# violetdenim/c3dgs

Hardware: AMD Instinct MI355X
Metric: raster views/sec fwd+bwd @1920x1080 (higher is better)
Workload: dtype f32; 1 GPU; BASELINE.json configs[2]: synth-v1 3M Gaussians, SH deg 3, indexed-camera rasterizer (QAT inner loop), mark_visible+fwd+bwd, 1 view/step/GPU; gaussians=3000000, width=1920, height=1080, sh_codebook=304096, gaussian_codebook=754096, parallelism=replicas x1

## Files before the change

c3dgs_amd/_lib.py:

```python
import ctypes as C
import os

_HERE = os.path.dirname(os.path.abspath(__file__))
LIB_PATH = os.environ.get("C3DGS_LIB_PATH") or os.path.join(_HERE, "libc3dgs_hip.so")

_f32p = C.POINTER(C.c_float)
_i64p = C.POINTER(C.c_int64)
_i32p = C.POINTER(C.c_int32)
_u8p = C.POINTER(C.c_uint8)

RESIZE_FN = C.CFUNCTYPE(C.c_void_p, C.c_void_p, C.c_size_t)


class RasterParams(C.Structure):
    _fields_ = [
        ("P", C.c_int32), ("D", C.c_int32), ("M", C.c_int32), ("W", C.c_int32), ("H", C.c_int32),
        ("SHS", C.c_int32), ("GS", C.c_int32),
        ("background", C.c_void_p), ("means3D", C.c_void_p), ("sh", C.c_void_p), ("colors_precomp", C.c_void_p),
        ("opacities", C.c_void_p), ("scales", C.c_void_p), ("scale_factors", C.c_void_p), ("rotations", C.c_void_p),
        ("cov3D_precomp", C.c_void_p), ("sh_indices", C.c_void_p), ("g_indices", C.c_void_p),
        ("viewmatrix", C.c_void_p), ("projmatrix", C.c_void_p), ("campos", C.c_void_p),
        ("tan_fovx", C.c_float), ("tan_fovy", C.c_float), ("scale_modifier", C.c_float),
        ("prefiltered", C.c_int32), ("clamp_color", C.c_int32), ("debug", C.c_int32),
    ]
# ... 10 lines not shown
        "total_bytes", "splat", "depth_keys", "depth_keys_sorted", "depth_order",
        "sorted_offsets", "inst_offset", "rects", "clamped", "scan_temp", "scan_temp_bytes", "block_base", "depth_base")]


class BinningLayout(C.Structure):
    _fields_ = [(n, C.c_size_t) for n in (
        "total_bytes", "keys_unsorted", "values_unsorted", "keys_sorted", "point_list", "sort_temp", "sort_temp_bytes")]


class StageTime(C.Structure):
    _fields_ = [("name", C.c_char * 32), ("total_ms", C.c_double), ("count", C.c_int64)]


class ImageLayout(C.Structure):
    _fields_ = [(n, C.c_size_t) for n in ("total_bytes", "final_T", "n_contrib", "ranges", "tile_used", "tile_order")]


class QatParams(C.Structure):
    _fields_ = [("P", C.c_int32), ("GS", C.c_int32), ("SHS", C.c_int32), ("M", C.c_int32),
                ("xyz", C.c_void_p), ("opacity", C.c_void_p), ("scaling_factor", C.c_void_p), ("scaling", C.c_void_p),
                ("rotation", C.c_void_p), ("features_dc", C.c_void_p), ("features_rest", C.c_void_p), ("state", C.c_void_p),
                ("observer_enabled", C.c_int32 * 6), ("fake_quant_enabled", C.c_int32 * 6),
                ("half_xyz", C.c_int32), ("averaging_constant", C.c_float)]


class AdamTensor(C.Structure):
    _fields_ = [("param", C.c_void_p), ("grad", C.c_void_p), ("exp_avg", C.c_void_p), ("exp_avg_sq", C.c_void_p), ("n", C.c_int64),
                ("step_size", C.c_float), ("bias_correction2_sqrt", C.c_float)]


# ... 56 lines not shown
    "c3dgs_qat_points": (C.c_int, [C.POINTER(QatParams)] + [_vp] * 10),
    "c3dgs_qat_points_backward": (C.c_int, [C.POINTER(QatParams)] + [_vp] * 11),
    "c3dgs_qat_quantize": (C.c_int, [C.POINTER(QatParams), C.c_int32] + [_vp] * 7),
    "c3dgs_fake_quantize": (C.c_int, [C.c_int64, _vp, _vp, C.c_int32, C.c_int32, C.c_float, _vp, _vp, _vp]),
    "c3dgs_fake_quantize_backward": (C.c_int, [C.c_int64, _vp, _vp, C.c_int32, _vp, _vp, _vp]),
    "c3dgs_debug_lane_counters": (C.c_int, [C.POINTER(C.c_uint64), _vp]),
    "c3dgs_debug_sort_times": (C.c_int, [C.POINTER(C.c_uint64)]),
    "c3dgs_debug_gather_probe": (C.c_int, [C.c_int32, C.c_int64, _vp, _vp, _vp, _vp]),
    "c3dgs_debug_sort_temp_bytes": (C.c_size_t, [C.c_int32, C.c_int64, C.c_int32]),
    "c3dgs_debug_sort_pairs": (C.c_int, [C.c_int32, C.c_int64, C.c_int32, _vp, _vp, _vp, _vp, _vp, C.c_size_t, _vp]),
    "c3dgs_debug_tile_sort_temp_bytes": (C.c_size_t, [C.c_int32, C.c_int64]),
    "c3dgs_debug_tile_sort_pairs": (C.c_int, [C.c_int32, C.c_int64, _vp, _vp, _vp, _vp, _vp, C.c_size_t, _vp]),
    "c3dgs_get_geom_layout": (C.c_int, [C.c_int32, C.POINTER(GeomLayout)]),
    "c3dgs_get_binning_layout": (C.c_int, [C.c_int32, C.c_int32, C.c_int32, C.POINTER(BinningLayout)]),
    "c3dgs_get_image_layout": (C.c_int, [C.c_int32, C.c_int32, C.POINTER(ImageLayout)]),
    "c3dgs_backward_workspace_bytes": (C.c_size_t, [C.c_int32, C.c_int32]),
    "c3dgs_profile_enable": (C.c_int, [C.c_int]),
    "c3dgs_profile_only": (C.c_int, [C.c_char_p]),
    "c3dgs_profile_read": (C.c_int, [C.POINTER(StageTime), C.c_int]),
    "c3dgs_last_error": (C.c_char_p, []),
    "c3dgs_abi_version": (C.c_int, []),
    "c3dgs_abs_accumulate": (C.c_int, [C.c_int64, C.c_void_p, C.c_void_p, C.c_void_p]),
}

_lib = None


def lib():
    global _lib
    if _lib is None:
# ... 32 lines not shown
```

c3dgs_amd/csrc/binning.hip:

```cpp
#include "common.hpp"
#include <rocprim/device/device_radix_sort.hpp>
#include <rocprim/iterator/counting_iterator.hpp>

namespace c3dgs {

size_t scan_temp_bytes(int P)
{
    size_t a = 0, b = 0;
    (void)rocprim::radix_sort_pairs(nullptr, b, (const uint32_t*)nullptr, (uint32_t*)nullptr, (const uint32_t*)nullptr,
                                    (uint32_t*)nullptr, (size_t)P, 0u, 32u);
    size_t m = a > b ? a : b;
    const size_t os = onesweep_depth_temp_bytes(P);
    if (os > m) m = os;
    return m < 256 ? 256 : m;
}

size_t sort_temp_bytes(int R, int end_bit, int key_bytes)
{
    size_t bytes = 0;
    if (key_bytes == 4)
        (void)rocprim::radix_sort_pairs(nullptr, bytes, (const uint32_t*)nullptr, (uint32_t*)nullptr,
                                        (const uint32_t*)nullptr, (uint32_t*)nullptr, (size_t)R, 0u, (unsigned)end_bit);
    else
        (void)rocprim::radix_sort_pairs(nullptr, bytes, (const uint16_t*)nullptr, (uint16_t*)nullptr,
                                        (const uint32_t*)nullptr, (uint32_t*)nullptr, (size_t)R, 0u, (unsigned)end_bit);
    const size_t os = onesweep_tile_temp_bytes(R, end_bit, key_bytes);
    if (os > bytes) bytes = os;
    const size_t reuse = align_up((size_t)(R > 0 ? R : 1));
    if (reuse > bytes) bytes = reuse;
    return bytes < 256 ? 256 : bytes;
}

__global__ void __launch_bounds__(256)
gather_u64_kernel(int n, const uint32_t* __restrict__ idx, const uint2* __restrict__ src, uint2* __restrict__ dst)
{
    const int i = blockIdx.x * 256 + threadIdx.x;
    if (i < n) dst[i] = src[idx[i]];
}

size_t depth_sort_clear_bytes(int P)
{
    return (onesweep_enabled() && (size_t)P < ((size_t)1 << 30)) ? onesweep_depth_clear_bytes(P) : 0;
}
// ... 34 lines not shown
```

c3dgs_amd/csrc/c_abi.hip:

```cpp
#include "common.hpp"
#include <cstdlib>
#include <cstring>
#include <mutex>
#include <vector>

namespace c3dgs {

static thread_local std::string g_last_error;
void set_error(const std::string& msg) { g_last_error = msg; }

enum Stage { ST_MARK_VISIBLE, ST_PREPROCESS, ST_DEPTH_SORT, ST_SCAN, ST_DUPLICATE, ST_SORT, ST_RANGES, ST_RENDER_FWD, ST_ZERO_PARTIALS,
             ST_RENDER_BWD, ST_BWD_PREPROCESS, ST_WDIST, ST_VQ_ACC, ST_VQ_APPLY, ST_LOSS_FWD, ST_LOSS_BWD,
             ST_QAT_OBSERVE, ST_QAT_CODEBOOKS, ST_QAT_VISIBLE, ST_QAT_POINTS, ST_QAT_POINTS_BWD, ST_QAT_CODEBOOKS_BWD, ST_ADAM,
             ST_KNN_SORT, ST_KNN_BOUNDS, ST_KNN_QUERY, ST_COUNT };
static const char* kStageNames[ST_COUNT] = { "mark_visible", "preprocess", "depth_sort", "scan", "duplicate_with_keys", "sort",
                                             "identify_ranges", "render_forward", "zero_partials", "render_backward",
                                             "backward_preprocess", "weighted_distance", "vq_accumulate", "vq_apply", "l1_ssim_forward",
                                             "l1_ssim_backward", "qat_observe", "qat_codebooks", "qat_visible", "qat_points",
                                             "qat_points_backward", "qat_codebooks_backward", "adam_step",
                                             "knn_sort", "knn_bounds", "knn_query" };
struct ProfRec { int stage; hipEvent_t a, b; };
static std::mutex g_prof_mu;
static bool g_prof_on = false;
static int g_prof_only = -1;
// ... 176 lines not shown
    if (R > 0) {
        const int end_bit = tile_sort_end_bit(W, H);
        size_t tclear = tile_sort_clear_bytes(R, end_bit, b.key_bytes);
        if (tclear > b.sort_temp_bytes) tclear = 0;
        { StageTimer t_(ST_DUPLICATE, s); launch_duplicate_with_keys(P, g, b, gx, sort_err, b.sort_temp, tclear / 16, s); }
        C3DGS_STAGE("duplicate_with_keys", p.debug, s);
        { StageTimer t_(ST_SORT, s);
          C3DGS_HIP_TRY(run_tile_sort(b.sort_temp, b.sort_temp_bytes, b.keys_unsorted, b.keys_sorted, b.key_bytes, b.values_unsorted,
                                      b.point_list, R, end_bit, s, tclear != 0)); }
        C3DGS_STAGE("sort", p.debug, s);
        if (p.debug && onesweep_timed_out(s)) return fail(C3DGS_E_HIP, "tile sort: look-back timed out");
        { StageTimer t_(ST_RANGES, s); launch_identify_ranges(R, b.keys_sorted, b.key_bytes, img.ranges, sort_err, s); }
        C3DGS_STAGE("identify_ranges", p.debug, s);
    }
    { StageTimer t_(ST_RENDER_FWD, s);
      launch_render_forward(W, H, img, b.point_list, g.splat, p.background, out_color, (uint8_t*)b.sort_temp, sort_err, s); }
    C3DGS_STAGE("render_forward", p.debug, s);
    return C3DGS_OK;
}

static int backward_impl(const c3dgs_raster_params* pp, bool indexed, const int32_t* radii, const void* geom_buffer,
                         const void* binning_buffer, const void* image_buffer, int32_t R, const float* dL_dout_color,
                         c3dgs_resize_fn ws_resize, void* ws_user, const c3dgs_raster_grads* grads, void* stream_)
{
    if (int rc = validate(pp, indexed, true)) return rc;
    if (!grads) return fail(C3DGS_E_INVALID, "grads is NULL");
    c3dgs_raster_params p = *pp;
    if (!indexed) { p.sh_indices = nullptr; p.g_indices = nullptr; p.scale_factors = nullptr; }
    hipStream_t s = (hipStream_t)stream_;
    const int P = p.P, W = p.W, H = p.H;

// ... 30 lines not shown
    float* partials = (float*)ws_resize(ws_user, ws_bytes);
    if (!partials) return fail(C3DGS_E_ALLOC, "backward workspace allocation failed");

    const size_t r1 = (size_t)(R > 0 ? R : 1), p256 = ((size_t)P + 1023) / 1024 * 1024;
    uint8_t* touched = (uint8_t*)partials + align_up(r1 * PARTIAL_FLOATS * sizeof(float));
    uint32_t* tile_order = img.tile_order;
    uint32_t* live_ids = (uint32_t*)(touched + align_up(r1)) + 65536;
    uint32_t* live_slots = live_ids + p256;
    uint32_t* live_count = live_slots + p256;
    { StageTimer t_(ST_ZERO_PARTIALS, s);
      launch_backward_prep(R > 0 ? W : 0, H, img, tile_order, touched, align_up(r1) / 16, R > 0 ? nullptr : cb_zero,
                           R > 0 ? 0 : cb_zero16, s); }
    if (R > 0) {
        const BinPtrs b = bin_ptrs(const_cast<void*>(binning_buffer), R, W, H);
        { StageTimer t_(ST_RENDER_BWD, s);
          launch_render_backward(W, H, img, b.point_list, g.splat, g.block_base, p.background, dL_dout_color, partials, touched,
                                 (const uint8_t*)b.sort_temp, tile_order, cb_zero, cb_zero16, s); }
        C3DGS_STAGE("render_backward", p.debug, s);
    }
    { StageTimer t_(ST_BWD_PREPROCESS, s);
      launch_backward_preprocess(p, radii, g, partials, touched, live_count, live_ids, live_slots, *grads, s); }
    C3DGS_STAGE("backward_preprocess", p.debug, s);
    return C3DGS_OK;
}

}

using namespace c3dgs;

extern "C" {

const char* c3dgs_last_error(void) { return g_last_error.c_str(); }
// ... 132 lines not shown
    geom_layout(P, out);
    return C3DGS_OK;
}
int c3dgs_get_binning_layout(int32_t R, int32_t W, int32_t H, c3dgs_binning_layout* out)
{
    if (!out || R < 0 || W <= 0 || H <= 0) return fail(C3DGS_E_INVALID, "bad arguments");
    binning_layout(R, W, H, out);
    return C3DGS_OK;
}
int c3dgs_get_image_layout(int32_t W, int32_t H, c3dgs_image_layout* out)
{
    if (!out || W <= 0 || H <= 0) return fail(C3DGS_E_INVALID, "bad arguments");
    image_layout(W, H, out);
    return C3DGS_OK;
}
size_t c3dgs_backward_workspace_bytes(int32_t P, int32_t R)
{
    const size_t r = (size_t)(R > 0 ? R : 1), p256 = ((size_t)(P > 0 ? P : 1) + 1023) / 1024 * 1024;
    return align_up(r * PARTIAL_FLOATS * sizeof(float)) + align_up(r) + 65536 * sizeof(uint32_t) +
           (2 * p256 + p256 / 256) * sizeof(uint32_t) + 256;
}

int c3dgs_mark_visible(int32_t P, const float* means3D, const float* viewmatrix, const float* projmatrix, uint8_t* present,
                       void* stream)
{
    (void)projmatrix;
    if (P < 0) return fail(C3DGS_E_INVALID, "P must be >= 0");
    if (P == 0) return C3DGS_OK;
    if (!means3D || !viewmatrix || !present) return fail(C3DGS_E_INVALID, "means3D, viewmatrix and present are required");
    { StageTimer t_(ST_MARK_VISIBLE, (hipStream_t)stream); launch_mark_visible(P, means3D, viewmatrix, present, (hipStream_t)stream); }
// ... 427 lines not shown
```

c3dgs_amd/csrc/common.hpp:

```cpp
#pragma once
#include <hip/hip_runtime.h>
#include <cstdint>
#include <cstddef>
#include <cstdio>
#include <cstring>
#include <string>

#include "../../include/c3dgs_hip.h"

namespace c3dgs {

constexpr int TILE = 16;
constexpr int TILE_PIX = 256;
constexpr int SPLAT_F4 = 3;
constexpr int PARTIAL_FLOATS = 9;

void set_error(const std::string& msg);
inline int fail(int code, const std::string& msg) { set_error(msg); return code; }

#define C3DGS_HIP_TRY(expr)                                                                         \
    do {                                                                                            \
        hipError_t e__ = (expr);                                                                    \
        if (e__ != hipSuccess)                                                                      \
            return ::c3dgs::fail(C3DGS_E_HIP, std::string(#expr) + ": " + hipGetErrorString(e__));  \
// ... 70 lines not shown

inline void binning_layout(int R, int W, int H, c3dgs_binning_layout* L)
{
    size_t o = 0, r = (size_t)(R > 0 ? R : 1);
    const int end_bit = tile_sort_end_bit(W, H);
    const size_t kb = (size_t)tile_key_bytes(W, H);
    L->keys_unsorted = o;   o = align_up(o + r * kb);
    L->values_unsorted = o; o = align_up(o + r * 4);
    L->keys_sorted = o;     o = align_up(o + r * kb);
    L->point_list = o;      o = align_up(o + r * 4);
    L->sort_temp = o;       L->sort_temp_bytes = sort_temp_bytes((int)r, end_bit, (int)kb);
    o = align_up(o + L->sort_temp_bytes);
    L->total_bytes = o;
}

inline void image_layout(int W, int H, c3dgs_image_layout* L)
{
    size_t o = 0, n = (size_t)W * H, t = (size_t)tiles_x(W) * tiles_y(H);
    L->final_T = o;   o = align_up(o + n * 4);
    L->n_contrib = o; o = align_up(o + n * 4);
    L->ranges = o;    o = align_up(o + t * 8);
    L->tile_used = o; o = align_up(o + t * 4);
    L->tile_order = o; o = align_up(o + t * 4);
    L->total_bytes = o;
}

struct GeomPtrs {
    float4* splat; uint32_t* depth_keys; uint32_t* depth_keys_sorted;
    uint32_t* depth_order; uint2* sorted_offsets; uint32_t* inst_offset; uint16_t* rects;
    uint8_t* clamped; uint32_t* block_base; uint32_t* depth_base; void* scan_temp; size_t scan_temp_bytes;
    float4* gtab;
};
struct BinPtrs {
    void* keys_unsorted; uint32_t* values_unsorted; void* keys_sorted; uint32_t* point_list;
    void* sort_temp; size_t sort_temp_bytes; int key_bytes;
};
struct ImgPtrs { float* final_T; uint32_t* n_contrib; uint2* ranges; uint32_t* tile_used; uint32_t* tile_order; };

inline GeomPtrs geom_ptrs(void* base, int P)
{
    c3dgs_geom_layout L; geom_layout(P, &L);
    char* b = (char*)base;
    return { (float4*)(b + L.splat), (uint32_t*)(b + L.depth_keys), (uint32_t*)(b + L.depth_keys_sorted), (uint32_t*)(b + L.depth_order),
             (uint2*)(b + L.sorted_offsets), (uint32_t*)(b + L.inst_offset), (uint16_t*)(b + L.rects),
             (uint8_t*)(b + L.clamped), (uint32_t*)(b + L.block_base), (uint32_t*)(b + L.depth_base), (void*)(b + L.scan_temp),
             L.scan_temp_bytes, (float4*)(b + L.total_bytes) };
}
inline BinPtrs bin_ptrs(void* base, int R, int W, int H)
{
    c3dgs_binning_layout L; binning_layout(R, W, H, &L);
    char* b = (char*)base;
    return { (void*)(b + L.keys_unsorted), (uint32_t*)(b + L.values_unsorted), (void*)(b + L.keys_sorted),
             (uint32_t*)(b + L.point_list), (void*)(b + L.sort_temp), L.sort_temp_bytes, tile_key_bytes(W, H) };
}
inline ImgPtrs img_ptrs(void* base, int W, int H)
{
    c3dgs_image_layout L; image_layout(W, H, &L);
    char* b = (char*)base;
    return { (float*)(b + L.final_T), (uint32_t*)(b + L.n_contrib), (uint2*)(b + L.ranges), (uint32_t*)(b + L.tile_used),
             (uint32_t*)(b + L.tile_order) };
}

void launch_camera_from_pose(const float* pose, float inv_tan_x, float inv_tan_y, float* view, float* proj, float* campos, hipStream_t s);
void launch_mark_visible(int P, const float* means3D, const float* view, uint8_t* present, hipStream_t s);
void launch_mark_visible_pose(int P, const float* means3D, const float* pose7, uint8_t* present, hipStream_t s);
void launch_pack_codebook(const c3dgs_raster_params& p, float4* gtab, hipStream_t s);
void launch_preprocess(const c3dgs_raster_params& p, const GeomPtrs& g, int32_t* radii, uint2* ranges, const uint32_t* sort_err,
                       void* zero_span, size_t zero_n16, uint32_t* host_out, uint32_t host_seq, hipStream_t s);
void launch_depth_order_scan(int P, const GeomPtrs& g, hipStream_t s);
void launch_duplicate_with_keys(int P, const GeomPtrs& g, const BinPtrs& b, int grid_x, const uint32_t* sort_err,
                                void* zero_span, size_t zero_n16, hipStream_t s);
void launch_identify_ranges(int R, const void* keys_sorted, int key_bytes, uint2* ranges, const uint32_t* sort_err, hipStream_t s);
hipError_t run_depth_sort(void* temp, size_t temp_bytes, const uint32_t* kin, uint32_t* kout, const uint32_t* vin,
                          uint32_t* vout, int P, const uint2* rects, uint2* rects_sorted, hipStream_t s, bool ctrl_cleared = false,
                          bool rects_fit_bytes = false);
// ... 6 lines not shown
uint32_t* onesweep_error_word();
size_t onesweep_depth_temp_bytes(int P);
size_t onesweep_tile_temp_bytes(int R, int end_bit, int key_bytes = 2);
size_t onesweep_depth_clear_bytes(int P);
size_t onesweep_tile_clear_bytes(int R, int end_bit, int key_bytes);
hipError_t onesweep_depth_sort(void* temp, size_t temp_bytes, const uint32_t* kin, uint32_t* kout, const uint32_t* vin, uint32_t* vout,
                               int P, const uint2* gather_src, uint2* gather_dst, hipStream_t s, bool ctrl_cleared = false,
                               bool rects_fit_bytes = false);
hipError_t onesweep_tile_sort32(void* temp, size_t temp_bytes, const uint32_t* kin, uint32_t* kout, const uint32_t* vin, uint32_t* vout,
                                int R, int end_bit, hipStream_t s, bool ctrl_cleared = false);
hipError_t onesweep_tile_sort(void* temp, size_t temp_bytes, const uint16_t* kin, uint16_t* kout, const uint32_t* vin, uint32_t* vout,
                              int R, int end_bit, hipStream_t s, bool ctrl_cleared = false);
int os_read_times(unsigned long long* out512);
int read_lane_counters(unsigned long long* out16, hipStream_t s);
void launch_render_forward(int W, int H, const ImgPtrs& img, const uint32_t* point_list, const float4* splat,
                           const float* bg, float* out_color, uint8_t* qmask, const uint32_t* sort_err, hipStream_t s);
void launch_backward_prep(int W, int H, const ImgPtrs& img, uint32_t* tile_order, void* zero_a, size_t n16_a, void* zero_b,
                          size_t n16_b, hipStream_t s);
void launch_render_backward(int W, int H, const ImgPtrs& img, const uint32_t* point_list, const float4* splat,
                            const uint32_t* block_base, const float* bg, const float* dL_dpix, float* partials,
                            uint8_t* touched, const uint8_t* qmask, const uint32_t* tile_order, void* zero_span, size_t zero_n16,
                            hipStream_t s);
void launch_backward_preprocess(const c3dgs_raster_params& p, const int32_t* radii, const GeomPtrs& g,
                                float* partials, const uint8_t* touched, uint32_t* live_count, uint32_t* live_ids,
                                uint32_t* live_slots, const c3dgs_raster_grads& gr, hipStream_t s);
int launch_weighted_distance(int64_t N, int C, int K, const float* coefs, const int64_t* gather, const float* codebook,
                             float* out_dist, int64_t* out_idx, hipStream_t s, void* ws = nullptr, size_t ws_bytes = 0, int presplit = -1);
bool wd_presplit_supported(int C, int K, const float* coefs, const float* codebook, const void* ws, size_t ws_bytes);
int launch_vq_apply_split(int K, int D, float* S, float* codebook, float* entry_importance, float decay, float alpha, float eps,
                          int scale_normalize, void* ws, size_t ws_bytes, int parity, hipStream_t s);
void launch_vq_seed_words(int K, int D, void* ws, hipStream_t s);
uint32_t* vq_next_absmax_word(int K, int D, void* ws, int parity);
size_t wd_ws_bytes(int64_t N, int C, int K);
int launch_wd_debug_scores(int64_t N, int C, int K, const float* coefs, const float* codebook, float* scores, void* ws, size_t ws_bytes,
                           float* out_dist, int64_t* out_idx, hipStream_t s);
void launch_vq_accumulate(int64_t B, int K, int D, const float* x, const float* w, const int64_t* gather,
// ... 49 lines not shown
```

c3dgs_amd/csrc/render.hip:

```cpp
#include "common.hpp"
#include <algorithm>

namespace c3dgs {

constexpr int BATCH = 256;

__device__ unsigned long long g_lane_counters[16];

#ifndef C3DGS_BWD_ABLATE
#define C3DGS_BWD_ABLATE 0
#endif
#ifdef C3DGS_BWD_TIMING
#define BT_STAMP(var) const unsigned long long var = __builtin_readcyclecounter();
#else
#define BT_STAMP(var)
#endif
#ifdef C3DGS_COUNT_LANES
struct LaneCount {
    unsigned long long pairs = 0, slots = 0, lanes = 0, live = 0, half = 0, blk = 0, lists = 0, aux = 0;
    int nA = 0, nB = 0, nb[4] = { 0, 0, 0, 0 };
    __device__ void pair(bool real, unsigned long long used, unsigned long long aux_mask)
    {
        slots++;
        if (!real) return;
// ... 106 lines not shown
#pragma unroll
    for (int o = 1; o < 64; o <<= 1) { const uint32_t v = __shfl_up(incl, o); if (lane >= o) incl += v; }
    if (lane == 63) s_w[wave] = incl;
    __syncthreads();
    uint32_t off = 0;
    for (int w = 0; w < wave; w++) off += s_w[w];
    s_cnt[t] = off + incl - c;
    __syncthreads();
    for (int i = t; i < T; i += 1024) order[atomicAdd(&s_cnt[1023 - min(work(i) >> 3, 1023u)], 1u)] = (uint32_t)i;
}

__global__ void __launch_bounds__(256)
render_forward_kernel(int W, int H, int gx, int T, const uint2* __restrict__ ranges, const uint32_t* __restrict__ point_list,
                      const float4* __restrict__ splat, const float* __restrict__ bg, float* __restrict__ out_color,
                      float* __restrict__ final_T, uint32_t* __restrict__ n_contrib, uint32_t* __restrict__ tile_used,
                      uint8_t* __restrict__ qmask, const uint32_t* __restrict__ sort_err)
{
    const int tile = tile_of_block(blockIdx.x, T);
    if (tile >= T || (blockIdx.x >> 3) >= ((T + 7) >> 3)) return;
    __shared__ float4 s_ab[2][BATCH + 1][2];
    __shared__ float s_c[2][BATCH + 1];
    __shared__ uint32_t s_list[4][BATCH + 8];
    __shared__ int s_wdone[2][4];
    __shared__ unsigned long long s_mask[2][4][4];
    __shared__ uint32_t s_used;
    constexpr uint32_t REC_BYTES = 32, BUF_BYTES = (BATCH + 1) * REC_BYTES;

    const int tid = threadIdx.x, wave = tid >> 6, lane = tid & 63;
    const int tx = tile % gx, ty = tile / gx;
    const int px = tx * TILE + (wave & 1) * 8 + (lane & 7);
    const int py = ty * TILE + (wave >> 1) * 8 + (lane >> 3);
    const bool inside = px < W && py < H;
    const float pxf = (float)px, pyf = (float)py;
    bool done = !inside;
    if (tid == 0) s_used = 0;
    if (tid < 2) { s_ab[tid][BATCH][0] = make_float4(0, 0, 0, 0); s_ab[tid][BATCH][1] = make_float4(0, 0, 0, 0); s_c[tid][BATCH] = 0.f; }
    const float tile_x0 = (float)(tx * TILE), tile_y0 = (float)(ty * TILE);

    const bool poisoned = *sort_err != 0u;
    const uint2 range = poisoned ? make_uint2(0u, 0u) : ranges[tile];
    const int n = (int)(range.y - range.x);
    const int rounds = (n + BATCH - 1) / BATCH;

    float Tr = 1.0f, C0 = 0.f, C1 = 0.f, C2 = 0.f;
    uint32_t last_contributor = 0;
    constexpr uint32_t NO_ENTRY = 0xffffffffu;
#ifdef C3DGS_COUNT_LANES
    LaneCount lc;
#endif
    const char* rec_base = reinterpret_cast<const char*>(&s_ab[0][0][0]);
    const char* blue_base = reinterpret_cast<const char*>(&s_c[0][0]);

    float4 ra = make_float4(0, 0, 0, 0), rb = ra, rc = ra;
    if (tid < n) {
        const uint32_t id = point_list[range.x + tid];
        ra = splat[3 * (size_t)id]; rb = splat[3 * (size_t)id + 1]; rc = splat[3 * (size_t)id + 2];
    }
    for (int r = 0; r < rounds; r++) {
        const int buf = r & 1;
        const uint32_t qm = (r * BATCH + tid < n) ? quadrant_mask(ra, rb, tile_x0, tile_y0) : 0u;
        prescale_conic(ra, rb);
        s_ab[buf][tid][0] = ra; s_ab[buf][tid][1] = rb; s_c[buf][tid] = rc.x;
        if (r * BATCH + tid < n) qmask[range.x + r * BATCH + tid] = (uint8_t)qm;
#pragma unroll
        for (int q = 0; q < 4; q++) {
            const unsigned long long bm = __ballot((qm >> q) & 1u);
            if (lane == 0) s_mask[buf][q][wave] = bm;
        }
        const bool wave_done = __all(done);
        if (lane == 0) s_wdone[buf][wave] = wave_done;
        __syncthreads();
        if (s_wdone[buf][0] & s_wdone[buf][1] & s_wdone[buf][2] & s_wdone[buf][3]) break;
        const int nxt = (r + 1) * BATCH + tid;
        if (nxt < n) {
            const uint32_t id = point_list[range.x + nxt];
            ra = splat[3 * (size_t)id]; rb = splat[3 * (size_t)id + 1]; rc = splat[3 * (size_t)id + 2];
        }
        if (wave_done) continue;
        int nw = 0;
        {
            const unsigned long long lt = (1ull << lane) - 1ull;
            const uint32_t buf_off = (uint32_t)buf * BUF_BYTES;
#pragma unroll
            for (int c = 0; c < 4; c++) {
                const unsigned long long m = uniform_u64(s_mask[buf][wave][c]);
                if ((m >> lane) & 1ull) s_list[wave][nw + (int)__popcll(m & lt)] = buf_off + (uint32_t)(c * 64 + lane) * REC_BYTES;
                nw += (int)__popcll(m);
            }
            if (lane < 8) s_list[wave][nw + lane] = buf_off + (uint32_t)BATCH * REC_BYTES;
            __builtin_amdgcn_fence(__ATOMIC_RELEASE, "wavefront");
            __builtin_amdgcn_wave_barrier();
            __builtin_amdgcn_fence(__ATOMIC_ACQUIRE, "wavefront");
// ... 16 lines not shown
                const bool stop = live_px && test_T < 0.0001f;
                const bool blend = live_px != stop;
                const float w = blend ? alpha * Tr : 0.f;
                C0 = fmaf(b.z, w, C0); C1 = fmaf(b.w, w, C1); C2 = fmaf(cblue, w, C2);
                Tr = blend ? test_T : Tr;
                last_off = blend ? e[g] : last_off;
                done = done || stop;
#ifdef C3DGS_COUNT_LANES
                lc.pair(k + g < nw, __ballot(blend), __ballot(hit));
#endif
            }
        }
#ifdef C3DGS_COUNT_LANES
        lc.end_list();
#endif
        if (last_off != NO_ENTRY) last_contributor = (uint32_t)(r * BATCH) + ((last_off - (uint32_t)buf * BUF_BYTES) >> 5) + 1u;
    }
    if (inside) {
        const size_t pix = (size_t)W * py + px, HW = (size_t)H * W;
        final_T[pix] = Tr;
        n_contrib[pix] = last_contributor;
        const float poison = poisoned ? __uint_as_float(0x7fc00000u) : 0.f;
        out_color[pix] = fmaf(Tr, bg[0], C0) + poison;
        out_color[HW + pix] = fmaf(Tr, bg[1], C1) + poison;
        out_color[2 * HW + pix] = fmaf(Tr, bg[2], C2) + poison;
    }
#ifdef C3DGS_COUNT_LANES
    lc.flush(0, lane);
#endif
    atomicMax(&s_used, last_contributor);
    __syncthreads();
    if (tid == 0) tile_used[tile] = s_used;
}

void launch_render_forward(int W, int H, const ImgPtrs& img, const uint32_t* point_list, const float4* splat,
                           const float* bg, float* out_color, uint8_t* qmask, const uint32_t* sort_err, hipStream_t s)
{
    const int gx = tiles_x(W), T = gx * tiles_y(H);
    const int grid = ((T + 7) / 8) * 8;
    render_forward_kernel<<<grid, 256, 0, s>>>(W, H, gx, T, img.ranges, point_list, splat, bg, out_color, img.final_T,
                                               img.n_contrib, img.tile_used, qmask, sort_err);
}

constexpr int NPART = PARTIAL_FLOATS;
constexpr int GROUP_G = 8;
constexpr int NCOL = 6;

template <int CTRL>
__device__ __forceinline__ float dpp_take(float v)
{
    return __int_as_float(__builtin_amdgcn_update_dpp(0, __float_as_int(v), CTRL, 0xf, 0xf, true));
}

template <int N, int CTRL>
__device__ __forceinline__ void transpose_reduce_step(float* v, bool hi)
{
// ... 35 lines not shown
    auto s1 = __builtin_amdgcn_permlane16_swap(__float_as_uint(o[1]), __float_as_uint(o[3]), false, false);
    auto s8 = __builtin_amdgcn_permlane16_swap(__float_as_uint(t8), __float_as_uint(t8), false, false);
    const float w0 = __uint_as_float(s0[0]) + __uint_as_float(s0[1]);
    const float w1 = __uint_as_float(s1[0]) + __uint_as_float(s1[1]);
    const float w8 = __uint_as_float(s8[0]) + __uint_as_float(s8[1]);
    auto s2 = __builtin_amdgcn_permlane32_swap(__float_as_uint(w0), __float_as_uint(w1), false, false);
    auto s9 = __builtin_amdgcn_permlane32_swap(__float_as_uint(w8), __float_as_uint(w8), false, false);
    total = __uint_as_float(s2[0]) + __uint_as_float(s2[1]);
    ninth = __uint_as_float(s9[0]) + __uint_as_float(s9[1]);
}

#ifndef C3DGS_BWD_WPE
#define C3DGS_BWD_WPE 5
#endif
__global__ void __launch_bounds__(256) __attribute__((amdgpu_waves_per_eu(C3DGS_BWD_WPE, C3DGS_BWD_WPE)))
render_backward_kernel(int W, int H, int gx, int T, const uint2* __restrict__ ranges, const uint32_t* __restrict__ tile_used,
                       const uint32_t* __restrict__ point_list, const float4* __restrict__ splat,
                       const uint32_t* __restrict__ block_base, const float* __restrict__ bg, const float* __restrict__ final_Ts,
                       const uint32_t* __restrict__ n_contrib, const float* __restrict__ dL_dpixels,
                       float* __restrict__ partials, uint8_t* __restrict__ touched, const uint8_t* __restrict__ qmask,
                       const uint32_t* __restrict__ tile_order, uint4* __restrict__ zero_span, size_t zero_n16)
{
    if (zero_n16) {
        const size_t per = (zero_n16 + gridDim.x - 1) / gridDim.x, z0 = (size_t)blockIdx.x * per, z1 = min(z0 + per, zero_n16);
        for (size_t i = z0 + threadIdx.x; i < z1; i += 256) zero_span[i] = make_uint4(0u, 0u, 0u, 0u);
    }
    if ((int)blockIdx.x >= T) return;
    BT_STAMP(bt_begin)
#ifdef C3DGS_BWD_TIMING
    unsigned long long bt_stage = 0, bt_list = 0, bt_loop = 0, bt_flush = 0, bt_s0 = 0, bt_s1 = 0, bt_s2 = 0, bt_s3 = 0, bt_f0 = 0;
#endif
    const int tile = (int)tile_order[blockIdx.x];
    __shared__ float4 s_ab[BATCH + 1][2];
    __shared__ float s_c[BATCH + 1];
    __shared__ uint32_t s_slot[BATCH];
// ... 2 lines not shown
    __shared__ float s_part[2][BATCH][NPART];
    constexpr uint32_t REC_BYTES = 32;
    const char* rec_base = reinterpret_cast<const char*>(&s_ab[0][0]);
    const char* blue_base = reinterpret_cast<const char*>(&s_c[0]);

    const int tid = threadIdx.x, wave = tid >> 6, lane = tid & 63;
    const int tx = tile % gx, ty = tile / gx;
    const int px = tx * TILE + (wave & 1) * 8 + (lane & 7);
    const int py = ty * TILE + (wave >> 1) * 8 + (lane >> 3);
    const bool inside = px < W && py < H;
    const float pxf = (float)px, pyf = (float)py;
    const size_t pix = (size_t)W * py + px, HW = (size_t)H * W;

    const uint2 range = ranges[tile];
    const int n = (int)(range.y - range.x);
    const int used = min(n, (int)tile_used[tile]);
    if (used <= 0) return;
    const int rounds = (used + BATCH - 1) / BATCH;
    if (tid == 0) { s_ab[BATCH][0] = make_float4(0, 0, 0, 0); s_ab[BATCH][1] = make_float4(0, 0, 0, 0); s_c[BATCH] = 0.f; }
    for (int q = tid; q < 4 * (BATCH / 2 + GROUP_G); q += 256) (&s_list[0][0])[q] = (uint32_t)BATCH * REC_BYTES;

    const float T_final = inside ? final_Ts[pix] : 0.f;
    float Tr = T_final;
    const int last_contributor = inside ? (int)n_contrib[pix] : 0;
    float dpx0 = 0.f, dpx1 = 0.f, dpx2 = 0.f;
    if (inside) { dpx0 = dL_dpixels[pix]; dpx1 = dL_dpixels[HW + pix]; dpx2 = dL_dpixels[2 * HW + pix]; }
    float Sd = T_final * (bg[0] * dpx0 + bg[1] * dpx1 + bg[2] * dpx2);
    int wave_last = last_contributor;
#pragma unroll
    for (int o = 32; o > 0; o >>= 1) wave_last = max(wave_last, __shfl_xor(wave_last, o));
    wave_last = __builtin_amdgcn_readfirstlane(wave_last);
    const int beta = ((lane >> 2) & 1) * 4 + (lane & 1) * 2 + ((lane >> 1) & 1);
    const int my_m = ((lane >> 3) & 1) * 4 + ((lane >> 4) & 1) * 2 + ((lane >> 5) & 1);
#ifdef C3DGS_COUNT_LANES
    LaneCount lc;
#endif

    uint32_t next_id = 0u, next_qm = 0u;
    {
        const int p0 = used - 1 - tid;
        if (p0 >= 0) { next_id = point_list[range.x + p0]; next_qm = qmask[range.x + p0]; }
    }
    BT_STAMP(bt_pro)
    for (int r = 0; r < rounds; r++) {
        BT_STAMP(bt0)
        __syncthreads();
        BT_STAMP(btA)
        const int mypos = used - 1 - (r * BATCH + tid);
        uint32_t qm = 0u;
        if (mypos >= 0) {
#if C3DGS_BWD_ABLATE & 16
            const uint32_t id = (range.x + (uint32_t)mypos) & 0x1fffffu;
#elif C3DGS_BWD_ABLATE & 2
            const uint32_t id = next_id & 4095u;
#else
            const uint32_t id = next_id;
#endif
            qm = next_qm;
            float4 a = splat[3 * (size_t)id], b = splat[3 * (size_t)id + 1];
            const float4 c = splat[3 * (size_t)id + 2];
            prescale_conic(a, b);
            const uint32_t off = __float_as_uint(c.y), lo = __float_as_uint(c.z), hi = __float_as_uint(c.w);
            const int x0 = lo & 0xffff, y0 = lo >> 16, x1 = hi & 0xffff;
#if C3DGS_BWD_ABLATE & 18
            s_slot[tid] = range.x + (uint32_t)mypos;
            (void)off; (void)x0; (void)y0; (void)x1;
#else
            s_slot[tid] = block_base[id >> 8] + off + (uint32_t)((ty - y0) * (x1 - x0) + (tx - x0));
#endif
            s_ab[tid][0] = a; s_ab[tid][1] = b; s_c[tid] = c.x;
        }
        {
            const int npos = mypos - BATCH;
            if (npos >= 0) { next_id = point_list[range.x + npos]; next_qm = qmask[range.x + npos]; }
        }
#pragma unroll
        for (int q = 0; q < 4; q++) {
            const unsigned long long bm = __ballot((qm >> q) & 1u);
            if (lane == 0) s_mask[q][wave] = bm;
        }
        BT_STAMP(btB)
#pragma unroll
        for (int w = 0; w < 2; w++)
#pragma unroll
            for (int q = 0; q < NPART; q++) s_part[w][tid][q] = 0.f;
        BT_STAMP(btC)
        __syncthreads();
        BT_STAMP(bt1)
#ifdef C3DGS_BWD_TIMING
// ... 153 lines not shown
int read_lane_counters(unsigned long long* out16, hipStream_t s)
{
    static const unsigned long long zeros[16] = { 0 };
    if (hipStreamSynchronize(s) != hipSuccess) return 1;
    if (hipMemcpyFromSymbol(out16, HIP_SYMBOL(g_lane_counters), sizeof(zeros)) != hipSuccess) return 1;
    return hipMemcpyToSymbol(HIP_SYMBOL(g_lane_counters), zeros, sizeof(zeros)) != hipSuccess;
}

void launch_backward_prep(int W, int H, const ImgPtrs& img, uint32_t* tile_order, void* zero_a, size_t n16_a, void* zero_b,
                          size_t n16_b, hipStream_t s)
{
    const int T = (W > 0 && H > 0 && tile_order) ? tiles_x(W) * tiles_y(H) : 0;
    const size_t n16 = n16_a + n16_b;
    if (T <= 0 && n16 == 0) return;
    const unsigned fill = n16 ? (unsigned)std::min<size_t>((n16 + 1023) / 1024, 1024) : 0u;
    backward_prep_kernel<<<1 + fill, 1024, 0, s>>>(T, img.tile_used, tile_order, (uint4*)zero_a, n16_a, (uint4*)zero_b, n16_b);
}

void launch_render_backward(int W, int H, const ImgPtrs& img, const uint32_t* point_list, const float4* splat,
                            const uint32_t* block_base, const float* bg, const float* dL_dpix, float* partials,
                            uint8_t* touched, const uint8_t* qmask, const uint32_t* tile_order, void* zero_span, size_t zero_n16,
                            hipStream_t s)
{
    const int gx = tiles_x(W), T = gx * tiles_y(H);
    const int grid = ((T + 7) / 8) * 8;
    render_backward_kernel<<<grid, 256, 0, s>>>(W, H, gx, T, img.ranges, img.tile_used, point_list, splat, block_base, bg, img.final_T,
                                                img.n_contrib, dL_dpix, partials, touched, qmask, tile_order, (uint4*)zero_span,
                                                zero_span ? zero_n16 : 0);
}

}
```

include/c3dgs_hip.h:

```cpp
#ifndef C3DGS_HIP_H
#define C3DGS_HIP_H

#include <stddef.h>
#include <stdint.h>

#ifdef __cplusplus
extern "C" {
#endif

#define C3DGS_ABI_VERSION 4

enum {
    C3DGS_OK = 0,
    C3DGS_E_INVALID = 1,
    C3DGS_E_HIP = 2,
    C3DGS_E_ALLOC = 3
};

typedef void* (*c3dgs_resize_fn)(void* user, size_t bytes);

typedef struct c3dgs_raster_params {
    int32_t P;
    int32_t D;
    int32_t M;
// ... 227 lines not shown
size_t c3dgs_debug_tile_sort_temp_bytes(int32_t tiles, int64_t n);
int c3dgs_debug_tile_sort_pairs(int32_t tiles, int64_t n, const void* keys_in, void* keys_out, const uint32_t* values_in,
                                uint32_t* values_out, void* temp, size_t temp_bytes, void* stream);

int c3dgs_debug_sort_times(uint64_t* out );

int c3dgs_debug_gather_probe(int32_t kind, int64_t n, void* table, const uint32_t* index, uint32_t* out, void* stream);

int c3dgs_debug_lane_counters(uint64_t* out , void* stream);

int c3dgs_get_geom_layout(int32_t P, c3dgs_geom_layout* out);
int c3dgs_get_binning_layout(int32_t R, int32_t W, int32_t H, c3dgs_binning_layout* out);
int c3dgs_get_image_layout(int32_t W, int32_t H, c3dgs_image_layout* out);
size_t c3dgs_backward_workspace_bytes(int32_t P, int32_t R);

typedef struct c3dgs_stage_time {
    char name[32];
    double total_ms;
    int64_t count;
} c3dgs_stage_time;
int c3dgs_profile_enable(int on);
int c3dgs_profile_only(const char* stage_name);
int c3dgs_profile_read(c3dgs_stage_time* out, int capacity);

const char* c3dgs_last_error(void);
int c3dgs_abi_version(void);

#ifdef __cplusplus
}
#endif
// ... 2 lines not shown
```

Measured before the change: 598.6 views/s.

## Compact per-tile splat lists in forward pass to skip dead entries in backward

The forward render kernel now writes a compacted per-tile list of splat ids and quadrant masks holding only entries whose quadrant mask is nonzero. It also records per-pixel and per-tile last-contributor indices in compacted coordinates. The backward render kernel iterates over this compacted list instead of the full point list, so splats that touch no quadrant of the tile are not processed in the backward pass. The cost is extra ballots, rank computation and scattered global writes in the forward pass, plus extra image buffer space for the compacted counters.

```diff
diff --git a/c3dgs_amd/_lib.py b/c3dgs_amd/_lib.py
--- a/c3dgs_amd/_lib.py
+++ b/c3dgs_amd/_lib.py
@@ -48,6 +48,10 @@
 
 class ImageLayout(C.Structure):
     _fields_ = [(n, C.c_size_t) for n in ("total_bytes", "final_T", "n_contrib", "ranges", "tile_used", "tile_order")]
+
+
+class CompactLayout(C.Structure):
+    _fields_ = [(n, C.c_size_t) for n in ("cqm", "cid", "tile_used_c", "n_contrib_c")]
 
 
 class QatParams(C.Structure):
@@ -134,6 +138,7 @@
     "c3dgs_get_geom_layout": (C.c_int, [C.c_int32, C.POINTER(GeomLayout)]),
     "c3dgs_get_binning_layout": (C.c_int, [C.c_int32, C.c_int32, C.c_int32, C.POINTER(BinningLayout)]),
     "c3dgs_get_image_layout": (C.c_int, [C.c_int32, C.c_int32, C.POINTER(ImageLayout)]),
+    "c3dgs_get_compact_layout": (C.c_int, [C.c_int32, C.c_int32, C.c_int32, C.POINTER(CompactLayout)]),
     "c3dgs_backward_workspace_bytes": (C.c_size_t, [C.c_int32, C.c_int32]),
     "c3dgs_profile_enable": (C.c_int, [C.c_int]),
     "c3dgs_profile_only": (C.c_int, [C.c_char_p]),
diff --git a/c3dgs_amd/csrc/binning.hip b/c3dgs_amd/csrc/binning.hip
--- a/c3dgs_amd/csrc/binning.hip
+++ b/c3dgs_amd/csrc/binning.hip
@@ -26,7 +26,7 @@
                                         (const uint32_t*)nullptr, (uint32_t*)nullptr, (size_t)R, 0u, (unsigned)end_bit);
     const size_t os = onesweep_tile_temp_bytes(R, end_bit, key_bytes);
     if (os > bytes) bytes = os;
-    const size_t reuse = align_up((size_t)(R > 0 ? R : 1));
+    const size_t reuse = compact_layout(R, 1, 1).bin_bytes;
     if (reuse > bytes) bytes = reuse;
     return bytes < 256 ? 256 : bytes;
 }
diff --git a/c3dgs_amd/csrc/c_abi.hip b/c3dgs_amd/csrc/c_abi.hip
--- a/c3dgs_amd/csrc/c_abi.hip
+++ b/c3dgs_amd/csrc/c_abi.hip
@@ -214,7 +214,7 @@
         C3DGS_STAGE("identify_ranges", p.debug, s);
     }
     { StageTimer t_(ST_RENDER_FWD, s);
-      launch_render_forward(W, H, img, b.point_list, g.splat, p.background, out_color, (uint8_t*)b.sort_temp, sort_err, s); }
+      launch_render_forward(W, H, img, b.point_list, g.splat, p.background, out_color, compact_ptrs(b, R, W, H), sort_err, s); }
     C3DGS_STAGE("render_forward", p.debug, s);
     return C3DGS_OK;
 }
@@ -275,8 +275,8 @@
     if (R > 0) {
         const BinPtrs b = bin_ptrs(const_cast<void*>(binning_buffer), R, W, H);
         { StageTimer t_(ST_RENDER_BWD, s);
-          launch_render_backward(W, H, img, b.point_list, g.splat, g.block_base, p.background, dL_dout_color, partials, touched,
-                                 (const uint8_t*)b.sort_temp, tile_order, cb_zero, cb_zero16, s); }
+          launch_render_backward(W, H, img, g.splat, g.block_base, p.background, dL_dout_color, partials, touched,
+                                 compact_ptrs(b, R, W, H), tile_order, cb_zero, cb_zero16, s); }
         C3DGS_STAGE("render_backward", p.debug, s);
     }
     { StageTimer t_(ST_BWD_PREPROCESS, s);
@@ -439,6 +439,15 @@
     image_layout(W, H, out);
     return C3DGS_OK;
 }
+int c3dgs_get_compact_layout(int32_t R, int32_t W, int32_t H, c3dgs_compact_layout* out)
+{
+    if (!out || R < 0 || W <= 0 || H <= 0) return fail(C3DGS_E_INVALID, "bad arguments");
+    c3dgs_binning_layout BL; binning_layout(R, W, H, &BL);
+    const CompactLayout C = compact_layout(R, W, H);
+    out->cqm = BL.sort_temp + C.cqm; out->cid = BL.sort_temp + C.cid;
+    out->tile_used_c = C.tile_used_c; out->n_contrib_c = C.n_contrib_c;
+    return C3DGS_OK;
+}
 size_t c3dgs_backward_workspace_bytes(int32_t P, int32_t R)
 {
     const size_t r = (size_t)(R > 0 ? R : 1), p256 = ((size_t)(P > 0 ? P : 1) + 1023) / 1024 * 1024;
diff --git a/c3dgs_amd/csrc/common.hpp b/c3dgs_amd/csrc/common.hpp
--- a/c3dgs_amd/csrc/common.hpp
+++ b/c3dgs_amd/csrc/common.hpp
@@ -108,6 +108,10 @@
     L->total_bytes = o;
 }
 
+inline size_t compact_image_bytes(int W, int H)
+{
+    return align_up((size_t)tiles_x(W) * tiles_y(H) * 4) + align_up((size_t)W * H * 4);
+}
 inline void image_layout(int W, int H, c3dgs_image_layout* L)
 {
     size_t o = 0, n = (size_t)W * H, t = (size_t)tiles_x(W) * tiles_y(H);
@@ -116,7 +120,19 @@
     L->ranges = o;    o = align_up(o + t * 8);
     L->tile_used = o; o = align_up(o + t * 4);
     L->tile_order = o; o = align_up(o + t * 4);
-    L->total_bytes = o;
+    L->total_bytes = o + compact_image_bytes(W, H);
+}
+
+struct CompactLayout { size_t cqm, cid, bin_bytes; size_t tile_used_c, n_contrib_c; };
+inline CompactLayout compact_layout(int R, int W, int H)
+{
+    const size_t r = (size_t)(R > 0 ? R : 1), t = (size_t)tiles_x(W) * tiles_y(H);
+    c3dgs_image_layout IL; image_layout(W, H, &IL);
+    CompactLayout C;
+    C.cqm = 0; C.cid = align_up(r); C.bin_bytes = C.cid + align_up(r * 4);
+    C.tile_used_c = IL.tile_order + align_up(t * 4);
+    C.n_contrib_c = C.tile_used_c + align_up(t * 4);
+    return C;
 }
 
 struct GeomPtrs {
@@ -129,7 +145,9 @@
     void* keys_unsorted; uint32_t* values_unsorted; void* keys_sorted; uint32_t* point_list;
     void* sort_temp; size_t sort_temp_bytes; int key_bytes;
 };
-struct ImgPtrs { float* final_T; uint32_t* n_contrib; uint2* ranges; uint32_t* tile_used; uint32_t* tile_order; };
+struct ImgPtrs { float* final_T; uint32_t* n_contrib; uint2* ranges; uint32_t* tile_used; uint32_t* tile_order;
+                 uint32_t* tile_used_c; uint32_t* n_contrib_c; };
+struct CompactPtrs { uint8_t* cqm; uint32_t* cid; };
 
 inline GeomPtrs geom_ptrs(void* base, int P)
 {
@@ -150,9 +168,15 @@
 inline ImgPtrs img_ptrs(void* base, int W, int H)
 {
     c3dgs_image_layout L; image_layout(W, H, &L);
+    const CompactLayout C = compact_layout(0, W, H);
     char* b = (char*)base;
     return { (float*)(b + L.final_T), (uint32_t*)(b + L.n_contrib), (uint2*)(b + L.ranges), (uint32_t*)(b + L.tile_used),
-             (uint32_t*)(b + L.tile_order) };
+             (uint32_t*)(b + L.tile_order), (uint32_t*)(b + C.tile_used_c), (uint32_t*)(b + C.n_contrib_c) };
+}
+inline CompactPtrs compact_ptrs(const BinPtrs& bp, int R, int W, int H)
+{
+    const CompactLayout C = compact_layout(R, W, H);
+    return { (uint8_t*)bp.sort_temp + C.cqm, (uint32_t*)((char*)bp.sort_temp + C.cid) };
 }
 
 void launch_camera_from_pose(const float* pose, float inv_tan_x, float inv_tan_y, float* view, float* proj, float* campos, hipStream_t s);
@@ -189,12 +213,12 @@
 int os_read_times(unsigned long long* out512);
 int read_lane_counters(unsigned long long* out16, hipStream_t s);
 void launch_render_forward(int W, int H, const ImgPtrs& img, const uint32_t* point_list, const float4* splat,
-                           const float* bg, float* out_color, uint8_t* qmask, const uint32_t* sort_err, hipStream_t s);
+                           const float* bg, float* out_color, const CompactPtrs& cl, const uint32_t* sort_err, hipStream_t s);
 void launch_backward_prep(int W, int H, const ImgPtrs& img, uint32_t* tile_order, void* zero_a, size_t n16_a, void* zero_b,
                           size_t n16_b, hipStream_t s);
-void launch_render_backward(int W, int H, const ImgPtrs& img, const uint32_t* point_list, const float4* splat,
+void launch_render_backward(int W, int H, const ImgPtrs& img, const float4* splat,
                             const uint32_t* block_base, const float* bg, const float* dL_dpix, float* partials,
-                            uint8_t* touched, const uint8_t* qmask, const uint32_t* tile_order, void* zero_span, size_t zero_n16,
+                            uint8_t* touched, const CompactPtrs& cl, const uint32_t* tile_order, void* zero_span, size_t zero_n16,
                             hipStream_t s);
 void launch_backward_preprocess(const c3dgs_raster_params& p, const int32_t* radii, const GeomPtrs& g,
                                 float* partials, const uint8_t* touched, uint32_t* live_count, uint32_t* live_ids,
diff --git a/c3dgs_amd/csrc/render.hip b/c3dgs_amd/csrc/render.hip
--- a/c3dgs_amd/csrc/render.hip
+++ b/c3dgs_amd/csrc/render.hip
@@ -144,7 +144,8 @@
 render_forward_kernel(int W, int H, int gx, int T, const uint2* __restrict__ ranges, const uint32_t* __restrict__ point_list,
                       const float4* __restrict__ splat, const float* __restrict__ bg, float* __restrict__ out_color,
                       float* __restrict__ final_T, uint32_t* __restrict__ n_contrib, uint32_t* __restrict__ tile_used,
-                      uint8_t* __restrict__ qmask, const uint32_t* __restrict__ sort_err)
+                      uint32_t* __restrict__ n_contrib_c, uint32_t* __restrict__ tile_used_c, uint8_t* __restrict__ cqm,
+                      uint32_t* __restrict__ cid, const uint32_t* __restrict__ sort_err)
 {
     const int tile = tile_of_block(blockIdx.x, T);
     if (tile >= T || (blockIdx.x >> 3) >= ((T + 7) >> 3)) return;
@@ -153,7 +154,10 @@
     __shared__ uint32_t s_list[4][BATCH + 8];
     __shared__ int s_wdone[2][4];
     __shared__ unsigned long long s_mask[2][4][4];
-    __shared__ uint32_t s_used;
+    __shared__ __attribute__((aligned(4))) uint8_t s_live[2][4];
+    __shared__ uint32_t s_used, s_used_c;
+    static_assert(sizeof(s_ab) + sizeof(s_c) + sizeof(s_list) + sizeof(s_wdone) + sizeof(s_mask) + sizeof(s_live) + 2 * sizeof(uint32_t)
+                      <= 18 * 1280, "render_forward: more than 18 LDS granules = six workgroups per CU instead of seven");
     constexpr uint32_t REC_BYTES = 32, BUF_BYTES = (BATCH + 1) * REC_BYTES;
 
     const int tid = threadIdx.x, wave = tid >> 6, lane = tid & 63;
@@ -163,7 +167,7 @@
     const bool inside = px < W && py < H;
     const float pxf = (float)px, pyf = (float)py;
     bool done = !inside;
-    if (tid == 0) s_used = 0;
+    if (tid == 0) { s_used = 0; s_used_c = 0; }
     if (tid < 2) { s_ab[tid][BATCH][0] = make_float4(0, 0, 0, 0); s_ab[tid][BATCH][1] = make_float4(0, 0, 0, 0); s_c[tid][BATCH] = 0.f; }
     const float tile_x0 = (float)(tx * TILE), tile_y0 = (float)(ty * TILE);
 
@@ -173,7 +177,8 @@
     const int rounds = (n + BATCH - 1) / BATCH;
 
     float Tr = 1.0f, C0 = 0.f, C1 = 0.f, C2 = 0.f;
-    uint32_t last_contributor = 0;
+    uint32_t last_contributor = 0, last_contributor_c = 0;
+    uint32_t n_live = 0;
     constexpr uint32_t NO_ENTRY = 0xffffffffu;
 #ifdef C3DGS_COUNT_LANES
     LaneCount lc;
@@ -182,8 +187,9 @@
     const char* blue_base = reinterpret_cast<const char*>(&s_c[0][0]);
 
     float4 ra = make_float4(0, 0, 0, 0), rb = ra, rc = ra;
+    uint32_t id = 0u;
     if (tid < n) {
-        const uint32_t id = point_list[range.x + tid];
+        id = point_list[range.x + tid];
         ra = splat[3 * (size_t)id]; rb = splat[3 * (size_t)id + 1]; rc = splat[3 * (size_t)id + 2];
     }
     for (int r = 0; r < rounds; r++) {
@@ -191,21 +197,34 @@
         const uint32_t qm = (r * BATCH + tid < n) ? quadrant_mask(ra, rb, tile_x0, tile_y0) : 0u;
         prescale_conic(ra, rb);
         s_ab[buf][tid][0] = ra; s_ab[buf][tid][1] = rb; s_c[buf][tid] = rc.x;
-        if (r * BATCH + tid < n) qmask[range.x + r * BATCH + tid] = (uint8_t)qm;
 #pragma unroll
         for (int q = 0; q < 4; q++) {
             const unsigned long long bm = __ballot((qm >> q) & 1u);
             if (lane == 0) s_mask[buf][q][wave] = bm;
         }
+        const unsigned long long live = __ballot(qm != 0u);
+        const uint32_t rank = __builtin_amdgcn_mbcnt_hi((uint32_t)(live >> 32), __builtin_amdgcn_mbcnt_lo((uint32_t)live, 0u));
+        if (lane == 0) s_live[buf][wave] = (uint8_t)__popcll(live);
         const bool wave_done = __all(done);
         if (lane == 0) s_wdone[buf][wave] = wave_done;
         __syncthreads();
         if (s_wdone[buf][0] & s_wdone[buf][1] & s_wdone[buf][2] & s_wdone[buf][3]) break;
+        const uint32_t cur_id = id;
         const int nxt = (r + 1) * BATCH + tid;
         if (nxt < n) {
-            const uint32_t id = point_list[range.x + nxt];
+            id = point_list[range.x + nxt];
             ra = splat[3 * (size_t)id]; rb = splat[3 * (size_t)id + 1]; rc = splat[3 * (size_t)id + 2];
         }
+        const uint32_t lv = __builtin_amdgcn_readfirstlane(*reinterpret_cast<const uint32_t*>(&s_live[buf][0]));
+        const uint32_t lv0 = lv & 0xffu, lv1 = (lv >> 8) & 0xffu, lv2 = (lv >> 16) & 0xffu, lv3 = lv >> 24;
+        const uint32_t wb1 = n_live + lv0, wb2 = wb1 + lv1, wb3 = wb2 + lv2;
+        const uint32_t wb0 = n_live;
+        auto wave_base = [&](uint32_t w) { return w == 0 ? wb0 : w == 1 ? wb1 : w == 2 ? wb2 : wb3; };
+        if (qm != 0u) {
+            const uint32_t ci = range.x + wave_base((uint32_t)wave) + rank;
+            cid[ci] = cur_id; cqm[ci] = (uint8_t)qm;
+        }
+        n_live = wb3 + lv3;
         if (wave_done) continue;
         int nw = 0;
         {
@@ -252,12 +271,19 @@
 #ifdef C3DGS_COUNT_LANES
         lc.end_list();
 #endif
-        if (last_off != NO_ENTRY) last_contributor = (uint32_t)(r * BATCH) + ((last_off - (uint32_t)buf * BUF_BYTES) >> 5) + 1u;
+        if (last_off != NO_ENTRY) {
+            const uint32_t j = (last_off - (uint32_t)buf * BUF_BYTES) >> 5;
+            last_contributor = (uint32_t)(r * BATCH) + j + 1u;
+            const uint32_t c = j >> 6;
+            const unsigned long long lv_c = s_mask[buf][0][c] | s_mask[buf][1][c] | s_mask[buf][2][c] | s_mask[buf][3][c];
+            last_contributor_c = wave_base(c) + (uint32_t)__popcll(lv_c & ((1ull << (j & 63u)) - 1ull)) + 1u;
+        }
     }
     if (inside) {
         const size_t pix = (size_t)W * py + px, HW = (size_t)H * W;
         final_T[pix] = Tr;
         n_contrib[pix] = last_contributor;
+        n_contrib_c[pix] = last_contributor_c;
         const float poison = poisoned ? __uint_as_float(0x7fc00000u) : 0.f;
         out_color[pix] = fmaf(Tr, bg[0], C0) + poison;
         out_color[HW + pix] = fmaf(Tr, bg[1], C1) + poison;
@@ -267,17 +293,18 @@
     lc.flush(0, lane);
 #endif
     atomicMax(&s_used, last_contributor);
+    atomicMax(&s_used_c, last_contributor_c);
     __syncthreads();
-    if (tid == 0) tile_used[tile] = s_used;
+    if (tid == 0) { tile_used[tile] = s_used; tile_used_c[tile] = s_used_c; }
 }
 
 void launch_render_forward(int W, int H, const ImgPtrs& img, const uint32_t* point_list, const float4* splat,
-                           const float* bg, float* out_color, uint8_t* qmask, const uint32_t* sort_err, hipStream_t s)
+                           const float* bg, float* out_color, const CompactPtrs& cl, const uint32_t* sort_err, hipStream_t s)
 {
     const int gx = tiles_x(W), T = gx * tiles_y(H);
     const int grid = ((T + 7) / 8) * 8;
     render_forward_kernel<<<grid, 256, 0, s>>>(W, H, gx, T, img.ranges, point_list, splat, bg, out_color, img.final_T,
-                                               img.n_contrib, img.tile_used, qmask, sort_err);
+                                               img.n_contrib, img.tile_used, img.n_contrib_c, img.tile_used_c, cl.cqm, cl.cid, sort_err);
 }
 
 constexpr int NPART = PARTIAL_FLOATS;
@@ -343,11 +370,11 @@
 #define C3DGS_BWD_WPE 5
 #endif
 __global__ void __launch_bounds__(256) __attribute__((amdgpu_waves_per_eu(C3DGS_BWD_WPE, C3DGS_BWD_WPE)))
-render_backward_kernel(int W, int H, int gx, int T, const uint2* __restrict__ ranges, const uint32_t* __restrict__ tile_used,
-                       const uint32_t* __restrict__ point_list, const float4* __restrict__ splat,
+render_backward_kernel(int W, int H, int gx, int T, const uint2* __restrict__ ranges, const uint32_t* __restrict__ tile_used_c,
+                       const uint32_t* __restrict__ cid, const float4* __restrict__ splat,
                        const uint32_t* __restrict__ block_base, const float* __restrict__ bg, const float* __restrict__ final_Ts,
-                       const uint32_t* __restrict__ n_contrib, const float* __restrict__ dL_dpixels,
-                       float* __restrict__ partials, uint8_t* __restrict__ touched, const uint8_t* __restrict__ qmask,
+                       const uint32_t* __restrict__ n_contrib_c, const float* __restrict__ dL_dpixels,
+                       float* __restrict__ partials, uint8_t* __restrict__ touched, const uint8_t* __restrict__ cqm,
                        const uint32_t* __restrict__ tile_order, uint4* __restrict__ zero_span, size_t zero_n16)
 {
     if (zero_n16) {
@@ -380,7 +407,7 @@
 
     const uint2 range = ranges[tile];
     const int n = (int)(range.y - range.x);
-    const int used = min(n, (int)tile_used[tile]);
+    const int used = min(n, (int)tile_used_c[tile]);
     if (used <= 0) return;
     const int rounds = (used + BATCH - 1) / BATCH;
     if (tid == 0) { s_ab[BATCH][0] = make_float4(0, 0, 0, 0); s_ab[BATCH][1] = make_float4(0, 0, 0, 0); s_c[BATCH] = 0.f; }
@@ -388,7 +415,7 @@
 
     const float T_final = inside ? final_Ts[pix] : 0.f;
     float Tr = T_final;
-    const int last_contributor = inside ? (int)n_contrib[pix] : 0;
+    const int last_contributor = inside ? (int)n_contrib_c[pix] : 0;
     float dpx0 = 0.f, dpx1 = 0.f, dpx2 = 0.f;
     if (inside) { dpx0 = dL_dpixels[pix]; dpx1 = dL_dpixels[HW + pix]; dpx2 = dL_dpixels[2 * HW + pix]; }
     float Sd = T_final * (bg[0] * dpx0 + bg[1] * dpx1 + bg[2] * dpx2);
@@ -405,7 +432,7 @@
     uint32_t next_id = 0u, next_qm = 0u;
     {
         const int p0 = used - 1 - tid;
-        if (p0 >= 0) { next_id = point_list[range.x + p0]; next_qm = qmask[range.x + p0]; }
+        if (p0 >= 0) { next_id = cid[range.x + p0]; next_qm = cqm[range.x + p0]; }
     }
     BT_STAMP(bt_pro)
     for (int r = 0; r < rounds; r++) {
@@ -415,9 +442,7 @@
         const int mypos = used - 1 - (r * BATCH + tid);
         uint32_t qm = 0u;
         if (mypos >= 0) {
-#if C3DGS_BWD_ABLATE & 16
-            const uint32_t id = (range.x + (uint32_t)mypos) & 0x1fffffu;
-#elif C3DGS_BWD_ABLATE & 2
+#if C3DGS_BWD_ABLATE & 2
             const uint32_t id = next_id & 4095u;
 #else
             const uint32_t id = next_id;
@@ -428,7 +453,7 @@
             prescale_conic(a, b);
             const uint32_t off = __float_as_uint(c.y), lo = __float_as_uint(c.z), hi = __float_as_uint(c.w);
             const int x0 = lo & 0xffff, y0 = lo >> 16, x1 = hi & 0xffff;
-#if C3DGS_BWD_ABLATE & 18
+#if C3DGS_BWD_ABLATE & 2
             s_slot[tid] = range.x + (uint32_t)mypos;
             (void)off; (void)x0; (void)y0; (void)x1;
 #else
@@ -438,7 +463,7 @@
         }
         {
             const int npos = mypos - BATCH;
-            if (npos >= 0) { next_id = point_list[range.x + npos]; next_qm = qmask[range.x + npos]; }
+            if (npos >= 0) { next_id = cid[range.x + npos]; next_qm = cqm[range.x + npos]; }
         }
 #pragma unroll
         for (int q = 0; q < 4; q++) {
@@ -622,18 +647,18 @@
     const size_t n16 = n16_a + n16_b;
     if (T <= 0 && n16 == 0) return;
     const unsigned fill = n16 ? (unsigned)std::min<size_t>((n16 + 1023) / 1024, 1024) : 0u;
-    backward_prep_kernel<<<1 + fill, 1024, 0, s>>>(T, img.tile_used, tile_order, (uint4*)zero_a, n16_a, (uint4*)zero_b, n16_b);
-}
-
-void launch_render_backward(int W, int H, const ImgPtrs& img, const uint32_t* point_list, const float4* splat,
+    backward_prep_kernel<<<1 + fill, 1024, 0, s>>>(T, img.tile_used_c, tile_order, (uint4*)zero_a, n16_a, (uint4*)zero_b, n16_b);
+}
+
+void launch_render_backward(int W, int H, const ImgPtrs& img, const float4* splat,
                             const uint32_t* block_base, const float* bg, const float* dL_dpix, float* partials,
-                            uint8_t* touched, const uint8_t* qmask, const uint32_t* tile_order, void* zero_span, size_t zero_n16,
+                            uint8_t* touched, const CompactPtrs& cl, const uint32_t* tile_order, void* zero_span, size_t zero_n16,
                             hipStream_t s)
 {
     const int gx = tiles_x(W), T = gx * tiles_y(H);
     const int grid = ((T + 7) / 8) * 8;
-    render_backward_kernel<<<grid, 256, 0, s>>>(W, H, gx, T, img.ranges, img.tile_used, point_list, splat, block_base, bg, img.final_T,
-                                                img.n_contrib, dL_dpix, partials, touched, qmask, tile_order, (uint4*)zero_span,
+    render_backward_kernel<<<grid, 256, 0, s>>>(W, H, gx, T, img.ranges, img.tile_used_c, cl.cid, splat, block_base, bg, img.final_T,
+                                                img.n_contrib_c, dL_dpix, partials, touched, cl.cqm, tile_order, (uint4*)zero_span,
                                                 zero_span ? zero_n16 : 0);
 }
 
diff --git a/include/c3dgs_hip.h b/include/c3dgs_hip.h
--- a/include/c3dgs_hip.h
+++ b/include/c3dgs_hip.h
@@ -265,6 +265,14 @@
 int c3dgs_get_image_layout(int32_t W, int32_t H, c3dgs_image_layout* out);
 size_t c3dgs_backward_workspace_bytes(int32_t P, int32_t R);
 
+typedef struct c3dgs_compact_layout {
+    size_t cqm;
+    size_t cid;
+    size_t tile_used_c;
+    size_t n_contrib_c;
+} c3dgs_compact_layout;
+int c3dgs_get_compact_layout(int32_t R, int32_t W, int32_t H, c3dgs_compact_layout* out);
+
 typedef struct c3dgs_stage_time {
     char name[32];
     double total_ms;
```

After: 619.1 views/s (median of 6 runs). 1.03x the previous value.
